# cshizhe/VLN-HAMT

Hardware: AMD Instinct MI355X
Metric: panorama-steps/sec, R2R proxy pretrain (36x768 views, 80-tok instr) (higher is better)
Workload: dtype bf16; 1 GPU; R2R 6-proxy-task pretrain step (fwd+bwd+clip+AdamW, dropout 0.1), fixed ViT features, R2R-canon model 174.8M params; per_gpu_batch=64, global_batch=64, txt_len=80, hist_len=5, views=36, task_mix=mlm:sap:sar:sprel:mrc:itm=5:1:1:1:2:2, parallelism=dp1, launch=hipGraph replay, dead_code_elimination=True

## Files before the change

include/hamt.h:

```cpp
#ifndef HAMT_H
#define HAMT_H

#include <stddef.h>
#include <stdint.h>

#ifdef __cplusplus
extern "C" {
#endif

#define HAMT_ABI_VERSION 2

typedef enum { HAMT_OK = 0, HAMT_ERR_ARG = -1, HAMT_ERR_UNSUPPORTED = -2, HAMT_ERR_LAUNCH = -3 } hamt_status;
typedef enum { HAMT_F32 = 0, HAMT_BF16 = 1,
               HAMT_U8G = 2,
               HAMT_F16 = 3 } hamt_dtype;
typedef enum { HAMT_PREC_BF16 = 0, HAMT_PREC_F32 = 1 } hamt_prec;

int hamt_version(void);
int hamt_last_error(char* buf, size_t n);
int hamt_last_kernel(char* buf, size_t n);
enum { HAMT_WS_GEMM_SPLITK = 0, HAMT_WS_COLSUM = 1, HAMT_WS_SUMSQ = 2, HAMT_WS_LN_BWD = 3, HAMT_WS_WGRAD_TABLE = 4, HAMT_WS_LNRED_TABLE = 5, HAMT_WS_VIS_EMBED_BWD = 6,
       HAMT_WS_EMBED_BWD = 7 ,
       HAMT_WS_OBJ_EMBED_BWD = 8, HAMT_WS_IMAGE_PREP = 9  };
size_t hamt_workspace_bytes(int op, const int* shape, int nshape);

enum {
  HAMT_EPI_BIAS = 1, HAMT_EPI_GELU = 2, HAMT_EPI_RELU = 4, HAMT_EPI_ACCUM = 8,
  HAMT_EPI_MUL_DGELU = 16, HAMT_EPI_MUL_DRELU = 32, HAMT_EPI_SAVE_PRE = 64,
  HAMT_EPI_GELU_GRAD = 128, HAMT_EPI_MUL_AUX = 256,
  HAMT_EPI_ADD_AUX = 512,
  HAMT_EPI_DROPOUT = 1024
};
typedef struct {
  int M, N, K;
  int lda, ldb, ldc, ldaux;
  int a_kmajor, b_kmajor;
  int dtype_a, dtype_b, dtype_c, dtype_aux;
  int prec;
  int epilogue;
  float alpha;
  int ka_rows, kb_rows;
  float p_drop;
  uint32_t call_id;
  const uint64_t* rng;
} hamt_gemm_desc;
int hamt_gemm(const hamt_gemm_desc* d, const void* A, const void* B, void* C, const float* bias,
              void* aux, void* stream);
int hamt_gemm_ksplit(const hamt_gemm_desc* d);
int hamt_gemm_ws(const hamt_gemm_desc* d, const void* A, const void* B, void* C, const float* bias,
                 void* aux, void* ws, size_t ws_bytes, void* stream);
int hamt_gemm_plan(const hamt_gemm_desc* d, size_t ws_bytes, char* name, size_t n);

int hamt_cast_pad_bf16(int R, int C, int Rpad, int Cpad, const float* x, int ldx, void* y, int ldy, void* stream);
int hamt_cast_transpose(int R, int C, const void* x, int ldx, int dtype_x, void* y, int ldy, int Rpad, void* stream);
int hamt_cast_pad_bf16_dropout(int R, int C, int Rpad, const float* x, int ldx, void* y, int ldy, float p, uint32_t call_id,
                               const uint64_t* rng, void* stream);

int hamt_smallk_wgrad(int M, int N, int K, const float* dy, int lddy, const float* x, int ldx, float* dW,
                      int accumulate, float* ws, void* stream);

typedef struct {
  const void* dy;
  const void* x;
  float* dw;
  float* db;
  int M, N, K, ldy, ldx, ldw;
  int accum_dw, accum_db;
  float* ss;
  int K_valid;
  float wire_scale;
  const void* dy2;
  const void* x2;
  int K2, ldy2, ldx2, K2_valid;
} hamt_wgrad_desc;
#define HAMT_WGRAD_TABLE_ENTRY 112
int hamt_wgrad_grouped(int n, const hamt_wgrad_desc* probs, void* table, size_t table_bytes, void* stream);
int hamt_wgrad_grouped_ex(int n, const hamt_wgrad_desc* probs, void* table, size_t table_bytes, int phase, void* stream);

int hamt_colsum(int M, int N, const void* x, int ldx, int dtype_x, float* out, int accumulate,
                float* ws, void* stream);

typedef struct {
  int B, heads, Sq, Sk, d_head;
  int ldq, ldk, ldv, ldo;
// ... 292 lines not shown
```

vln_hamt_amd/_lib.py:

```python
from __future__ import annotations

import ctypes as C
import os

_HERE = os.path.dirname(os.path.abspath(__file__))
LIB_PATH = os.path.join(_HERE, "libhamt_hip.so")

HAMT_F32, HAMT_BF16, HAMT_U8G, HAMT_F16 = 0, 1, 2, 3
PREC_BF16, PREC_F32 = 0, 1
EPI_BIAS, EPI_GELU, EPI_RELU, EPI_ACCUM, EPI_MUL_DGELU, EPI_MUL_DRELU, EPI_SAVE_PRE = 1, 2, 4, 8, 16, 32, 64
EPI_GELU_GRAD, EPI_MUL_AUX, EPI_ADD_AUX, EPI_DROPOUT = 128, 256, 512, 1024
SUMSQ_SPARSE = 2
OPT_ADAMW, OPT_ADAM, OPT_RMSPROP, OPT_SGD = 0, 1, 2, 3

vp, i32, u32, f32, sz = C.c_void_p, C.c_int, C.c_uint32, C.c_float, C.c_size_t


class GemmDesc(C.Structure):
    _fields_ = [("M", i32), ("N", i32), ("K", i32), ("lda", i32), ("ldb", i32), ("ldc", i32), ("ldaux", i32),
                ("a_kmajor", i32), ("b_kmajor", i32), ("dtype_a", i32), ("dtype_b", i32), ("dtype_c", i32),
                ("dtype_aux", i32), ("prec", i32), ("epilogue", i32), ("alpha", f32), ("ka_rows", i32), ("kb_rows", i32),
                ("p_drop", f32), ("call_id", u32), ("rng", C.c_void_p)]


# ... 47 lines not shown
    _fields_ = [("src", C.c_int32), ("left", C.c_int32), ("top", C.c_int32), ("width", C.c_int32), ("height", C.c_int32), ("flip", C.c_int32),
                ("zero", C.c_int32), ("order", C.c_int32), ("brightness", f32), ("contrast", f32), ("saturation", f32), ("reserved", C.c_int32)]


class ImagePrepDesc(C.Structure):
    _fields_ = [("n", i32), ("n_src", i32), ("H", i32), ("W", i32), ("layout", i32), ("ldy", i32), ("dtype_y", i32), ("Rpad", i32)]


RESAMPLE_BICUBIC, RESAMPLE_LANCZOS = 0, 1


class ImageResampleDesc(C.Structure):
    _fields_ = [(n, i32) for n in ("n", "H", "W", "OH", "OW", "x0", "y0", "w", "h", "filter", "kx", "ky")]


WGRAD_TABLE_ENTRY = 112


class WgradDesc(C.Structure):
    _fields_ = [("dy", vp), ("x", vp), ("dw", vp), ("db", vp), ("M", i32), ("N", i32), ("K", i32), ("ldy", i32),
                ("ldx", i32), ("ldw", i32), ("accum_dw", i32), ("accum_db", i32), ("ss", vp), ("K_valid", i32),
                ("wire_scale", f32), ("dy2", vp), ("x2", vp), ("K2", i32), ("ldy2", i32), ("ldx2", i32), ("K2_valid", i32)]


SIGNATURES = {
    "hamt_version": [],
    "hamt_last_error": [C.c_char_p, sz],
    "hamt_last_kernel": [C.c_char_p, sz],
    "hamt_workspace_bytes": [i32, C.POINTER(i32), i32],
    "hamt_gemm": [C.POINTER(GemmDesc), vp, vp, vp, vp, vp, vp],
    "hamt_gemm_ksplit": [C.POINTER(GemmDesc)],
    "hamt_gemm_ws": [C.POINTER(GemmDesc), vp, vp, vp, vp, vp, vp, sz, vp],
    "hamt_gemm_plan": [C.POINTER(GemmDesc), sz, C.c_char_p, sz],
    "hamt_cast_pad_bf16": [i32, i32, i32, i32, vp, i32, vp, i32, vp],
    "hamt_cast_pad_bf16_dropout": [i32, i32, i32, vp, i32, vp, i32, f32, u32, vp, vp],
    "hamt_cast_transpose": [i32, i32, vp, i32, i32, vp, i32, i32, vp],
    "hamt_wgrad_grouped": [i32, C.POINTER(WgradDesc), vp, sz, vp],
    "hamt_wgrad_grouped_ex": [i32, C.POINTER(WgradDesc), vp, sz, i32, vp],
    "hamt_smallk_wgrad": [i32, i32, i32, vp, i32, vp, i32, vp, i32, vp, vp],
    "hamt_colsum": [i32, i32, vp, i32, i32, vp, i32, vp, vp],
    "hamt_attn_small_fwd": [C.POINTER(AttnDesc), vp, vp, vp, vp, vp, vp, vp, vp],
    "hamt_attn_small_bwd": [C.POINTER(AttnDesc), vp, vp, vp, vp, vp, vp, vp, vp, vp, vp, vp, vp, vp],
    "hamt_attn_cls_fwd": [C.POINTER(AttnDesc), vp, vp, vp, vp, vp],
    "hamt_attn_varlen_fwd": [C.POINTER(AttnDesc), vp, vp, vp, vp, vp, vp, vp, vp],
    "hamt_attn_varlen_bwd": [C.POINTER(AttnDesc), vp, vp, vp, vp, vp, vp, vp, vp, vp, vp, vp, vp],
    "hamt_attn_varlen_cross_fwd": [C.POINTER(AttnDesc), vp, vp, vp, vp, vp, C.c_int, vp, vp, vp, vp, vp, vp],
    "hamt_attn_varlen_cross_bwd": [C.POINTER(AttnDesc), vp, vp, vp, vp, vp, C.c_int, vp, vp, vp, vp, vp, vp, vp, vp, vp, vp],
    "hamt_vis_embed_fwd": [C.POINTER(VisEmbedDesc)] + [vp] * 12,
    "hamt_vis_embed_bwd": [C.POINTER(VisEmbedDesc)] + [vp] * 18,
    "hamt_obj_embed_fwd": [C.POINTER(ObjEmbedDesc), C.POINTER(ObjEmbedParams)] + [vp] * 7,
    "hamt_obj_embed_bwd": [C.POINTER(ObjEmbedDesc), C.POINTER(ObjEmbedParams), C.POINTER(ObjEmbedGrads)] + [vp] * 10,
    "hamt_ln_fwd": [C.POINTER(LnDesc), vp, vp, vp, vp, vp, vp, vp, vp, vp, vp, vp],
    "hamt_ln_bwd": [C.POINTER(LnDesc), vp, vp, vp, vp, vp, vp, vp, vp, vp, vp, vp, vp, vp, vp],
    "hamt_ln_bwd_add": [C.POINTER(LnDesc), vp, vp, vp, vp, vp, vp, vp, vp, vp, vp, vp],
    "hamt_ln_bwd_reduce": [i32, i32, vp, vp, vp, vp, vp],
    "hamt_ln_bwd_reduce_grouped": [i32, vp, vp, sz, vp],
    "hamt_gather_rows": [i32, i32, vp, i32, vp, vp, i32, vp, i32, i32, vp],
    "hamt_scatter_add_rows": [i32, i32, vp, i32, i32, vp, vp, i32, vp],
    "hamt_scatter_add_rows_small": [i32, i32, vp, i32, i32, vp, i32, vp, vp, vp],
    "hamt_scatter_add_rows_ordered": [i32, i32, vp, i32, i32, vp, vp, i32, i32, vp, vp],
    "hamt_embed_sum_fwd": [i32, i32, i32, vp, vp, vp, vp, vp, vp],
    "hamt_embed_sum_bwd": [i32, i32, i32, i32, vp, vp, vp, vp, vp, vp, sz, vp],
    "hamt_mean_mid_fwd": [i32, i32, i32, vp, vp, vp],
    "hamt_mean_mid_bwd": [i32, i32, i32, vp, vp, vp],
    "hamt_mul_bcast_fwd": [i32, i32, i32, vp, vp, i32, vp, vp],
    "hamt_mul_bcast_bwd": [i32, i32, i32, vp, vp, i32, vp, vp, vp, vp],
# ... 67 lines not shown
        raise HamtError(f"{LIB_PATH} is missing: build it with `python vln_hamt_amd/csrc/build.py` "
                        "(there is no CPU/PyTorch fallback for the HAMT kernels)")
    import torch
    lib = C.CDLL(LIB_PATH)
    for name, args in SIGNATURES.items():
        fn = getattr(lib, name)
        fn.argtypes = args
        fn.restype = sz if name == "hamt_workspace_bytes" else i32
    if lib.hamt_version() != 2:
        raise HamtError("libhamt_hip.so ABI version mismatch")
    _lib = lib
    return lib


def last_error() -> str:
    buf = C.create_string_buffer(512)
    load().hamt_last_error(buf, 512)
    return buf.value.decode(errors="replace")


def last_kernel() -> str:
    buf = C.create_string_buffer(160)
    load().hamt_last_kernel(buf, 160)
    return buf.value.decode(errors="replace")


def gemm_plan(desc: GemmDesc, ws_bytes=None):
    buf = C.create_string_buffer(160)
    ks = load().hamt_gemm_plan(C.byref(desc), sz(-1).value if ws_bytes is None else ws_bytes, buf, 160)
    check(min(ks, 0), "hamt_gemm_plan")
    return ks, buf.value.decode(errors="replace")


def workspace_bytes(op: int, *shape) -> int:
    arr = (i32 * max(1, len(shape)))(*shape)
    return int(load().hamt_workspace_bytes(op, arr, len(shape)))


WS_GEMM_SPLITK, WS_COLSUM, WS_SUMSQ, WS_LN_BWD, WS_WGRAD_TABLE, WS_LNRED_TABLE, WS_VIS_EMBED_BWD, WS_EMBED_BWD, WS_OBJ_EMBED_BWD = range(9)
WS_IMAGE_PREP = 9


def check(rc: int, name: str):
    if rc != 0:
        raise HamtError(f"{name} failed (status {rc}): {last_error()}")
```

vln_hamt_amd/csrc/gemm.hip:

```cpp
#include "common.h"
#include "gemm_plan.h"

namespace {

struct GemmArgs {
  int M, N, K, lda, ldb;
  int ka_lim, kb_lim;
  int ldc, ldaux;
  int dtype_c, dtype_aux, epi;
  float alpha;
  const void* A;
  const void* B;
  void* C;
  const float* bias;
  void* aux;
};

__device__ __forceinline__ void epi_store(const GemmArgs& g, int row, int col, float acc) {
  if (row >= g.M || col >= g.N) return;
  float v = acc * g.alpha;
  if (g.epi & HAMT_EPI_BIAS) v += g.bias[col];
  size_t ia = (size_t)row * g.ldaux + col;
  if (g.epi & HAMT_EPI_SAVE_PRE) {
    if (g.dtype_aux == HAMT_BF16) ((bf16_t*)g.aux)[ia] = f2bf(v); else ((float*)g.aux)[ia] = v;
  }
  if (g.epi & HAMT_EPI_GELU) v = gelu_erf(v);
  if (g.epi & HAMT_EPI_GELU_GRAD) {
    float gg, dg;
    gelu_and_grad(v, gg, dg);
    v = gg;
    if (g.dtype_aux == HAMT_U8G) { const float d4[4] = {dg, 0.f, 0.f, 0.f}; ((uint8_t*)g.aux)[ia] = (uint8_t)(g8_pack4(d4) & 0xffu); }
    else if (g.dtype_aux == HAMT_BF16) ((bf16_t*)g.aux)[ia] = f2bf(dg); else ((float*)g.aux)[ia] = dg;
  }
  if (g.epi & HAMT_EPI_MUL_AUX)
    v *= g.dtype_aux == HAMT_U8G ? __builtin_fmaf((float)((const uint8_t*)g.aux)[ia], 0.005f, -0.13f)
                                 : ((g.dtype_aux == HAMT_BF16) ? bf2f(((const bf16_t*)g.aux)[ia]) : ((const float*)g.aux)[ia]);
  if (g.epi & HAMT_EPI_RELU) v = fmaxf(v, 0.0f);
  if (g.epi & (HAMT_EPI_MUL_DGELU | HAMT_EPI_MUL_DRELU)) {
    float h = (g.dtype_aux == HAMT_BF16) ? bf2f(((const bf16_t*)g.aux)[ia]) : ((const float*)g.aux)[ia];
    v *= (g.epi & HAMT_EPI_MUL_DGELU) ? dgelu_erf(h) : (h > 0.0f ? 1.0f : 0.0f);
  }
  if (g.epi & HAMT_EPI_ADD_AUX) v += (g.dtype_aux == HAMT_BF16) ? bf2f(((const bf16_t*)g.aux)[ia]) : ((const float*)g.aux)[ia];
  size_t ic = (size_t)row * g.ldc + col;
  if (g.dtype_c == HAMT_BF16) {
    bf16_t* c = (bf16_t*)g.C;
    if (g.epi & HAMT_EPI_ACCUM) v += bf2f(c[ic]);
    c[ic] = f2bf(v);
  } else if (g.dtype_c == HAMT_F16) {
    bf16_t* c = (bf16_t*)g.C;
    if (g.epi & HAMT_EPI_ACCUM) v += h2f(c[ic]);
    c[ic] = f2h(v);
  } else {
    float* c = (float*)g.C;
    if (g.epi & HAMT_EPI_ACCUM) v += c[ic];
    c[ic] = v;
  }
}

constexpr int F_BM = 64, F_BN = 64, F_BK = 32, F_LD = 64 + 16, F_NP = F_BK / 16;

template <bool KMAJOR>
__device__ __forceinline__ void f32_stage_load(const float* __restrict__ P, int ld, int r0, int rlim, int k0,
                                               int klim, int t, float (&v)[4]) {
  if (!KMAJOR) {
    int r = r0 + (t & 63), k = k0 + (t >> 6) * 4;
    if (r < rlim && k + 4 <= klim) {
      float4 x = *(const float4*)(P + (size_t)r * ld + k);
      v[0] = x.x; v[1] = x.y; v[2] = x.z; v[3] = x.w;
    } else {
#pragma unroll
      for (int j = 0; j < 4; ++j) v[j] = (r < rlim && k + j < klim) ? P[(size_t)r * ld + k + j] : 0.0f;
    }
  } else {
    int k = k0 + (t >> 4), r = r0 + (t & 15) * 4;
    if (k < klim && r + 4 <= rlim) {
      float4 x = *(const float4*)(P + (size_t)k * ld + r);
      v[0] = x.x; v[1] = x.y; v[2] = x.z; v[3] = x.w;
    } else {
#pragma unroll
      for (int j = 0; j < 4; ++j) v[j] = (k < klim && r + j < rlim) ? P[(size_t)k * ld + r + j] : 0.0f;
    }
  }
}
template <bool KMAJOR>
__device__ __forceinline__ void f32_stage_write(float* lds, int t, const float (&v)[4]) {
  if (!KMAJOR) {
    int r = t & 63, k = (t >> 6) * 4;
#pragma unroll
    for (int j = 0; j < 4; ++j) lds[(k + j) * F_LD + r] = v[j];
  } else {
    int k = t >> 4, r = (t & 15) * 4;
    *(float4*)(lds + k * F_LD + r) = make_float4(v[0], v[1], v[2], v[3]);
  }
}

template <bool A_KM, bool B_KM>
__global__ __launch_bounds__(256) void gemm_f32_kernel(GemmArgs g) {
  __shared__ __attribute__((aligned(16))) float lds[2][2][F_BK * F_LD];
  const int t = threadIdx.x, lane = t & 63, w = t >> 6, wm = w >> 1, wn = w & 1;
  const int tiles_n = (g.N + F_BN - 1) / F_BN;
  const int m0 = (blockIdx.x / tiles_n) * F_BM, n0 = (blockIdx.x % tiles_n) * F_BN;
  const float* A = (const float*)g.A;
  const float* B = (const float*)g.B;
  f32x4 acc[2][2];
#pragma unroll
  for (int i = 0; i < 2; ++i)
#pragma unroll
    for (int j = 0; j < 2; ++j) acc[i][j] = (f32x4){0.f, 0.f, 0.f, 0.f};

  float ra[F_NP][4], rb[F_NP][4];
  const int nk = (g.K + F_BK - 1) / F_BK;
#pragma unroll
  for (int h = 0; h < F_NP; ++h) {
    f32_stage_load<A_KM>(A, g.lda, m0, g.M, 16 * h, g.ka_lim, t, ra[h]);
    f32_stage_load<B_KM>(B, g.ldb, n0, g.N, 16 * h, g.kb_lim, t, rb[h]);
  }
#pragma unroll
  for (int h = 0; h < F_NP; ++h) {
    f32_stage_write<A_KM>(lds[0][0] + 16 * h * F_LD, t, ra[h]);
    f32_stage_write<B_KM>(lds[0][1] + 16 * h * F_LD, t, rb[h]);
  }
  __syncthreads();
  for (int kt = 0; kt < nk; ++kt) {
    const int cur = kt & 1;
    if (kt + 1 < nk) {
#pragma unroll
      for (int h = 0; h < F_NP; ++h) {
        f32_stage_load<A_KM>(A, g.lda, m0, g.M, (kt + 1) * F_BK + 16 * h, g.ka_lim, t, ra[h]);
        f32_stage_load<B_KM>(B, g.ldb, n0, g.N, (kt + 1) * F_BK + 16 * h, g.kb_lim, t, rb[h]);
      }
    }
    const float* As = lds[cur][0];
    const float* Bs = lds[cur][1];
#pragma unroll
    for (int s = 0; s < F_BK / 4; ++s) {
      const int kk = s * 4 + (lane >> 4);
      float a[2], b[2];
#pragma unroll
      for (int i = 0; i < 2; ++i) a[i] = As[kk * F_LD + wm * 32 + i * 16 + (lane & 15)];
#pragma unroll
      for (int j = 0; j < 2; ++j) b[j] = Bs[kk * F_LD + wn * 32 + j * 16 + (lane & 15)];
#pragma unroll
      for (int i = 0; i < 2; ++i)
#pragma unroll
        for (int j = 0; j < 2; ++j) acc[i][j] = __builtin_amdgcn_mfma_f32_16x16x4f32(a[i], b[j], acc[i][j], 0, 0, 0);
    }
    if (kt + 1 < nk) {
#pragma unroll
      for (int h = 0; h < F_NP; ++h) {
        f32_stage_write<A_KM>(lds[cur ^ 1][0] + 16 * h * F_LD, t, ra[h]);
        f32_stage_write<B_KM>(lds[cur ^ 1][1] + 16 * h * F_LD, t, rb[h]);
      }
    }
    __syncthreads();
  }
#pragma unroll
  for (int i = 0; i < 2; ++i)
#pragma unroll
    for (int j = 0; j < 2; ++j)
#pragma unroll
      for (int r = 0; r < 4; ++r)
        epi_store(g, m0 + wm * 32 + i * 16 + (lane >> 4) * 4 + r, n0 + wn * 32 + j * 16 + (lane & 15), acc[i][j][r]);
}

constexpr int H_BK = 32, H_PAD = 8;

template <typename T> struct Ld8;
template <> struct Ld8<float> {
  static __device__ __forceinline__ uint4 vec(const float* p) {
    float4 a = *(const float4*)p, b = *(const float4*)(p + 4);
    return make_uint4(pack_bf2(a.x, a.y), pack_bf2(a.z, a.w), pack_bf2(b.x, b.y), pack_bf2(b.z, b.w));
  }
  static __device__ __forceinline__ bf16_t one(const float* p) { return f2bf(*p); }
};
template <> struct Ld8<bf16_t> {
  static __device__ __forceinline__ uint4 vec(const bf16_t* p) { return *(const uint4*)p; }
  static __device__ __forceinline__ bf16_t one(const bf16_t* p) { return *p; }
};

template <typename T, bool KMAJOR, int R>
__device__ __forceinline__ uint4 h_stage_load(const T* __restrict__ P, int ld, int r0, int rlim, int k0, int klim, int c) {
  int r, k;
  const T* p;
  bool full;
  if (!KMAJOR) {
    r = r0 + (c >> 2); k = k0 + (c & 3) * 8;
    p = P + (size_t)r * ld + k;
    full = (r < rlim) && (k + 8 <= klim);
  } else {
    k = k0 + c / (R / 8); r = r0 + (c % (R / 8)) * 8;
    p = P + (size_t)k * ld + r;
    full = (k < klim) && (r + 8 <= rlim);
  }
  if (full) return Ld8<T>::vec(p);
  unsigned short e[8];
// ... 187 lines not shown
}

extern "C" int hamt_smallk_wgrad(int M, int N, int K, const float* dy, int lddy, const float* x, int ldx, float* dW, int accumulate,
                                 float* ws, void* stream) {
  HAMT_CHECK_ARG(dy && x && dW && ws && K >= 1 && K <= 8 && N >= 1 && M >= 0, "hamt_smallk_wgrad: bad argument (K <= 8)");
  hipStream_t s = as_stream(stream);
  int chunks = M >= 64 * 64 ? 64 : (M + 63) / 64;
  if (chunks < 1) chunks = 1;
  int rpc = (M + chunks - 1) / chunks;
  if (rpc < 1) rpc = 1;
  hipLaunchKernelGGL((smallk_wgrad_partial_kernel<8>), dim3((N + 63) / 64, chunks), dim3(256), 0, s, M, N, K, dy, lddy, x, ldx, ws, rpc);
  hamt_reduce_partials(chunks, N * K, ws, dW, accumulate, s);
  HAMT_CHECK_LAUNCH("hamt_smallk_wgrad");
  return HAMT_OK;
}

void hamt_gemm_fast_launch(const hamt_gemm_desc* d, const GemmPlan& p, const void* A, const void* B, void* C, const float* bias, void* aux,
                           float* ws, hipStream_t s);

void hamt_reduce_partials(int R, int N, const float* ws, float* out, int accumulate, hipStream_t s) {
  if (N % 4 == 0 && (((uintptr_t)ws | (uintptr_t)out) % 16) == 0) {
    const size_t n4 = (size_t)N / 4;
    const size_t b = (n4 + 255) / 256;
    hipLaunchKernelGGL(reduce_partials4_kernel, dim3((unsigned)(b > 4096 ? 4096 : b)), dim3(256), 0, s, R, n4, (size_t)N, ws, out, accumulate);
    return;
  }
  hipLaunchKernelGGL(reduce_partials_kernel, dim3((N + 63) / 64), dim3(256), 0, s, R, N, ws, out, accumulate);
}

static const GemmTuning& gemm_tuning() {
  static const GemmTuning t = [] {
    auto num = [](const char* name, int unset) { const char* v = getenv(name); return v ? atoi(v) : unset; };
    return GemmTuning{getenv("HAMT_NO_FAST") != nullptr, num("HAMT_FAST_BM", 0), num("HAMT_KS", 0), num("HAMT_KG", 0), num("HAMT_Q4", -1),
                      num("HAMT_P8", -1), num("HAMT_P8_BN", 0)};
  }();
  return t;
}

extern "C" int hamt_gemm_ksplit(const hamt_gemm_desc* d) { return d ? gemm_plan(*d, (size_t)-1, gemm_tuning()).ksplit : 1; }

extern "C" int hamt_gemm_plan(const hamt_gemm_desc* d, size_t ws_bytes, char* name, size_t n) {
  HAMT_CHECK_ARG(d && (name || n == 0), "hamt_gemm_plan: null pointer");
  const GemmPlan p = gemm_plan(*d, ws_bytes, gemm_tuning());
  if (n) gemm_plan_name(p, name, n);
  return p.ksplit;
}

extern "C" int hamt_gemm(const hamt_gemm_desc* d, const void* A, const void* B, void* C, const float* bias, void* aux,
                         void* stream) {
  return hamt_gemm_ws(d, A, B, C, bias, aux, nullptr, 0, stream);
}

extern "C" int hamt_gemm_ws(const hamt_gemm_desc* d, const void* A, const void* B, void* C, const float* bias, void* aux,
                            void* ws, size_t ws_bytes, void* stream) {
  HAMT_CHECK_ARG(d && A && B && C, "hamt_gemm: null pointer");
  HAMT_CHECK_ARG(d->M >= 0 && d->N >= 0 && d->K >= 0, "hamt_gemm: negative size");
  if (d->M == 0 || d->N == 0) return HAMT_OK;
  const int sa = d->dtype_a == HAMT_BF16 ? 2 : 4, sb = d->dtype_b == HAMT_BF16 ? 2 : 4;
  HAMT_CHECK_ARG((d->lda * sa) % 16 == 0 && (d->ldb * sb) % 16 == 0, "hamt_gemm: lda/ldb rows must be 16-byte aligned (lda=%d ldb=%d)", d->lda, d->ldb);
  HAMT_CHECK_ARG(((uintptr_t)A % 16) == 0 && ((uintptr_t)B % 16) == 0, "hamt_gemm: A/B must be 16-byte aligned");
  HAMT_CHECK_ARG(d->dtype_c == HAMT_F32 || d->dtype_c == HAMT_BF16 || d->dtype_c == HAMT_F16, "hamt_gemm: dtype_c = %d (C is fp32, bf16 or IEEE half)", d->dtype_c);
  HAMT_CHECK_ARG(d->dtype_c != HAMT_F16 || (d->epilogue & ~(HAMT_EPI_BIAS | HAMT_EPI_ACCUM)) == 0, "hamt_gemm: an IEEE-half C (HAMT_F16) takes the plain / bias / accumulate epilogues only");
  HAMT_CHECK_ARG((d->dtype_a == HAMT_F32 || d->dtype_a == HAMT_BF16) && (d->dtype_b == HAMT_F32 || d->dtype_b == HAMT_BF16), "hamt_gemm: operands are fp32 or bf16");
  HAMT_CHECK_ARG(!(d->epilogue & HAMT_EPI_BIAS) || bias, "hamt_gemm: EPI_BIAS without bias");
  HAMT_CHECK_ARG(!(d->epilogue & (HAMT_EPI_SAVE_PRE | HAMT_EPI_MUL_DGELU | HAMT_EPI_MUL_DRELU | HAMT_EPI_GELU_GRAD | HAMT_EPI_MUL_AUX | HAMT_EPI_ADD_AUX)) || aux, "hamt_gemm: epilogue needs aux");
  if (aux && d->dtype_aux == HAMT_U8G)
    HAMT_CHECK_ARG((d->epilogue & (HAMT_EPI_GELU_GRAD | HAMT_EPI_MUL_AUX)) && !(d->epilogue & (HAMT_EPI_SAVE_PRE | HAMT_EPI_MUL_DGELU | HAMT_EPI_MUL_DRELU | HAMT_EPI_ADD_AUX | HAMT_EPI_DROPOUT)),
                   "hamt_gemm: a HAMT_U8G aux is the gelu' image of HAMT_EPI_GELU_GRAD (without dropout) / HAMT_EPI_MUL_AUX only");
  const GemmPlan p = gemm_plan(*d, ws ? ws_bytes : 0, gemm_tuning());
  const bool fast = p.family != GEMM_F32 && p.family != GEMM_BF16;
  if (d->epilogue & HAMT_EPI_DROPOUT) {
    HAMT_CHECK_ARG(d->rng && d->p_drop >= 0.0f && d->p_drop < 1.0f, "hamt_gemm: EPI_DROPOUT needs rng and 0 <= p_drop < 1");
    HAMT_CHECK_ARG(fast, "hamt_gemm: EPI_DROPOUT is implemented by the bf16 MFMA path only (bf16 operands, K %% 64 == 0)");
  }
  const int ka = (d->ka_rows > 0 && d->ka_rows < d->K) ? d->ka_rows : d->K, kb = (d->kb_rows > 0 && d->kb_rows < d->K) ? d->kb_rows : d->K;
  GemmArgs g{d->M, d->N, d->K, d->lda, d->ldb, ka, kb, d->ldc, d->ldaux, d->dtype_c, d->dtype_aux, d->epilogue, d->alpha, A, B, C, bias, aux};
  hipStream_t s = as_stream(stream);
  char name[160];
  gemm_plan_name(p, name, sizeof(name));
  hamt_set_last_kernel("%s", name);
  if (fast) {
    hamt_gemm_fast_launch(d, p, A, B, C, bias, aux, (float*)ws, s);
    HAMT_CHECK_LAUNCH("hamt_gemm(fast)");
    return HAMT_OK;
  }
  if (d->prec == HAMT_PREC_F32) {
    HAMT_CHECK_ARG(d->dtype_a == HAMT_F32 && d->dtype_b == HAMT_F32, "hamt_gemm: PREC_F32 needs fp32 operands");
    int tiles = ((d->M + F_BM - 1) / F_BM) * ((d->N + F_BN - 1) / F_BN);
    if (!d->a_kmajor && !d->b_kmajor) hipLaunchKernelGGL((gemm_f32_kernel<false, false>), dim3(tiles), dim3(256), 0, s, g);
    else if (!d->a_kmajor && d->b_kmajor) hipLaunchKernelGGL((gemm_f32_kernel<false, true>), dim3(tiles), dim3(256), 0, s, g);
    else if (d->a_kmajor && !d->b_kmajor) hipLaunchKernelGGL((gemm_f32_kernel<true, false>), dim3(tiles), dim3(256), 0, s, g);
    else hipLaunchKernelGGL((gemm_f32_kernel<true, true>), dim3(tiles), dim3(256), 0, s, g);
  } else {
    static const bool use_tr = getenv("HAMT_NO_TR") == nullptr;
    static const int force_tile = getenv("HAMT_GEMM_TILE") ? atoi(getenv("HAMT_GEMM_TILE")) : 0;
    if (!d->a_kmajor && !d->b_kmajor) pick_types_bf16<false, false>(g, d->dtype_a, d->dtype_b, use_tr, force_tile, s);
    else if (!d->a_kmajor && d->b_kmajor) pick_types_bf16<false, true>(g, d->dtype_a, d->dtype_b, use_tr, force_tile, s);
    else if (d->a_kmajor && d->b_kmajor) pick_types_bf16<true, true>(g, d->dtype_a, d->dtype_b, use_tr, force_tile, s);
    else { hamt_set_error("hamt_gemm: a_kmajor=1,b_kmajor=0 is not used by the path"); return HAMT_ERR_UNSUPPORTED; }
  }
  HAMT_CHECK_LAUNCH("hamt_gemm");
  return HAMT_OK;
}

extern "C" int hamt_colsum(int M, int N, const void* x, int ldx, int dtype_x, float* out, int accumulate, float* ws,
                           void* stream) {
  HAMT_CHECK_ARG(x && out && ws && M >= 0 && N > 0, "hamt_colsum: bad argument");
  hipStream_t s = as_stream(stream);
  int chunks = M >= 64 * 64 ? 64 : (M + 63) / 64;
  if (chunks < 1) chunks = 1;
  int rpc = (M + chunks - 1) / chunks;
  if (rpc < 1) rpc = 1;
  dim3 grid((N + 63) / 64, chunks);
  if (dtype_x == HAMT_BF16) hipLaunchKernelGGL((colsum_partial_kernel<bf16_t>), grid, dim3(256), 0, s, M, N, (const bf16_t*)x, ldx, ws, rpc);
  else hipLaunchKernelGGL((colsum_partial_kernel<float>), grid, dim3(256), 0, s, M, N, (const float*)x, ldx, ws, rpc);
  hamt_reduce_partials(chunks, N, ws, out, accumulate, s);
  HAMT_CHECK_LAUNCH("hamt_colsum");
  return HAMT_OK;
}
```

vln_hamt_amd/csrc/gemm_plan.h:

```cpp
#pragma once
#include "../../include/hamt.h"
#include <stddef.h>
#include <stdio.h>

constexpr int PLAN_BN = 128, PLAN_BK = 64;

#define HAMT_EPIS_NARROW(X) X(0) X(HAMT_EPI_BIAS) X(HAMT_EPI_ACCUM)
#define HAMT_EPIS_P8(X) HAMT_EPIS_NARROW(X) X(HAMT_EPI_BIAS | HAMT_EPI_GELU_GRAD) X(HAMT_EPI_MUL_AUX)
#define HAMT_EPIS_P8_FWD(X)  \
  X(HAMT_EPI_BIAS | HAMT_EPI_ADD_AUX) X(HAMT_EPI_BIAS | HAMT_EPI_ADD_AUX | HAMT_EPI_DROPOUT) X(HAMT_EPI_BIAS | HAMT_EPI_GELU_GRAD | HAMT_EPI_DROPOUT) \
  X(HAMT_EPI_BIAS | HAMT_EPI_GELU) X(HAMT_EPI_BIAS | HAMT_EPI_GELU | HAMT_EPI_DROPOUT)
#define HAMT_EPIS_256(X) HAMT_EPIS_P8(X)  \
  X(HAMT_EPI_BIAS | HAMT_EPI_ADD_AUX) X(HAMT_EPI_BIAS | HAMT_EPI_ADD_AUX | HAMT_EPI_DROPOUT) X(HAMT_EPI_BIAS | HAMT_EPI_GELU_GRAD | HAMT_EPI_DROPOUT)
#define HAMT_EPIS_FAST(X) HAMT_EPIS_P8(X) HAMT_EPIS_P8_FWD(X)  \
  X(HAMT_EPI_BIAS | HAMT_EPI_GELU | HAMT_EPI_SAVE_PRE) X(HAMT_EPI_BIAS | HAMT_EPI_RELU) X(HAMT_EPI_MUL_DGELU)
#define HAMT_KG_VARIANTS(X) X(32, 2, 3) X(32, 3, 2) X(32, 2, 4) X(64, 2, 3) X(64, 3, 2) X(128, 2, 2)

#define HAMT_EPI_IS(E) if (e == (E)) return true;
static inline bool gemm_epi_narrow(int e) { HAMT_EPIS_NARROW(HAMT_EPI_IS) return false; }
static inline bool gemm_epi_256(int e) { HAMT_EPIS_256(HAMT_EPI_IS) return false; }
static inline bool gemm_epi_fast(int e) { HAMT_EPIS_FAST(HAMT_EPI_IS) return false; }
static inline bool gemm_epi_p8(int e, bool b_kmajor, int nb) {
  HAMT_EPIS_P8(HAMT_EPI_IS)
  if (!b_kmajor && nb == 4) { HAMT_EPIS_P8_FWD(HAMT_EPI_IS) }
  return false;
}
#undef HAMT_EPI_IS

struct GemmTuning {
  bool no_fast;
  int fast_bm;
  int ks;
  int kg;
  int q4, p8;
  int p8_bn;
};

enum GemmFamily { GEMM_F32, GEMM_BF16 , GEMM_FAST, GEMM_FAST256, GEMM_P8, GEMM_KG, GEMM_Q4 };

struct GemmPlan {
  GemmFamily family;
  int tile_rows;
  int p8_nb;
  int kg_groups, kg_depth;
  int epi;
  bool a_kmajor, b_kmajor;
  int ksplit;
};

static inline int gemm_plan_name(const GemmPlan& p, char* buf, size_t n) {
  const char *a = p.a_kmajor ? "true" : "false", *b = p.b_kmajor ? "true" : "false";
  switch (p.family) {
    case GEMM_F32: return snprintf(buf, n, "gemm_f32_kernel<%s, %s>", a, b);
    case GEMM_BF16: return snprintf(buf, n, "gemm_bf16_kernel<%s, %s, ...>", a, b);
    case GEMM_FAST: return snprintf(buf, n, "gemm_fast_kernel<%d, %d, %s, %s>", p.tile_rows, p.epi, a, b);
    case GEMM_FAST256: return snprintf(buf, n, "gemm_fast256_kernel<%d, %s, %s>", p.epi, a, b);
    case GEMM_P8: return snprintf(buf, n, "gemm_p8_kernel<%d, %s, %s, %d>", p.epi, a, b, p.p8_nb);
    case GEMM_KG: return snprintf(buf, n, "gemm_kg_kernel<%d, %d, %d, %s>", p.tile_rows, p.kg_groups, p.kg_depth, b);
    case GEMM_Q4: return snprintf(buf, n, "gemm_q4_kernel<%d, %s>", p.epi, b);
  }
  return -1;
}

static inline bool gemm_fast_eligible(const hamt_gemm_desc& d) {
  if (d.prec != HAMT_PREC_BF16 || d.dtype_a != HAMT_BF16 || d.dtype_b != HAMT_BF16) return false;
  if (d.a_kmajor && !d.b_kmajor) return false;
  if (d.K < 64 || d.M < 1 || d.N < 1) return false;
  if (d.K % 64 != 0) return false;
// ... 16 lines not shown
    if (bm == 32) return G == 2 && D == 3 ? GemmKg{32, 2, 3} : G == 3 ? GemmKg{32, 3, 2} : GemmKg{32, 2, 4};
    if (bm == 128) return {128, 2, 2};
    return G == 2 ? GemmKg{64, 2, 3} : GemmKg{64, 3, 2};
  }
  const int nk = d.K / PLAN_BK;
  if (nk < 12 || d.N > 1024) return {0, 0, 0};
  const long tn = (d.N + 127) / 128, t32 = (long)((d.M + 31) / 32) * tn, t64 = (long)((d.M + 63) / 64) * tn;
  if (nk >= 192 && t64 <= 128 && !(d.epilogue & ~HAMT_EPI_ACCUM) && d.dtype_c == HAMT_F32 && d.ldc == d.N) return {0, 0, 0};
  if (t32 <= 256) return {32, 2, 4};
  if (t64 <= 256 && nk >= 24) return {64, 3, 2};
  const long t128 = (long)((d.M + 127) / 128) * tn;
  if (t128 <= 256 && nk >= 36) return {128, 2, 2};
  return {0, 0, 0};
}

static inline int gemm_ksplit(const hamt_gemm_desc& d, size_t ws_bytes, const GemmTuning& t) {
  if (d.epilogue & ~HAMT_EPI_ACCUM) return 1;
  if (d.dtype_c != HAMT_F32 || d.ldc != d.N) return 1;
  if (!t.fast_bm && !t.ks && gemm_kg_variant(d, t).rows) return 1;
  const long tiles = (long)((d.M + 127) / 128) * ((d.N + 127) / 128);
  const int nk = d.K / PLAN_BK;
  int s;
  if (t.ks) s = t.ks > nk ? nk : t.ks;
  else {
    if (tiles >= 192 || nk < 16) return 1;
    s = (int)(384 / tiles);
    if (s > nk / 8) s = nk / 8;
    if (s > 16) s = 16;
  }
  while (s > 1 && (size_t)s * d.M * d.N * 4 > ws_bytes) --s;
  return s < 2 ? 1 : s;
}

static inline GemmPlan gemm_plan(const hamt_gemm_desc& d, size_t ws_bytes, const GemmTuning& t) {
  GemmPlan p{GEMM_BF16, 0, 0, 0, 0, -1, d.a_kmajor != 0, d.b_kmajor != 0, 1};
  if (t.no_fast || !gemm_fast_eligible(d)) {
    if (d.prec == HAMT_PREC_F32) p.family = GEMM_F32;
    return p;
  }
  const int e = d.epilogue, nk = d.K / PLAN_BK;
  const int ks = p.ksplit = gemm_ksplit(d, ws_bytes, t);
  const long t128 = (long)((d.M + 127) / 128) * ((d.N + 127) / 128), t64 = (long)((d.M + 63) / 64) * ((d.N + 127) / 128);
  const bool one_tile = ks == 1 && !t.fast_bm;
  if (one_tile && t.q4 != 0 && !d.a_kmajor && nk >= 3 && gemm_epi_narrow(e)) {
    if (t.q4 == 1 || (d.N <= 1024 && d.K >= 192 && t128 >= 120 && t128 <= 256)) { p.family = GEMM_Q4; p.epi = e; return p; }
  }
  if (one_tile && t.p8 != 0 && d.K >= 128 && !d.a_kmajor && (!d.b_kmajor || d.ldb >= 256)) {
    const long t256 = (long)((d.M + 255) / 256) * ((d.N + 255) / 256), t192 = (long)((d.M + 255) / 256) * ((d.N + 191) / 192);
    const double t_p8 = (double)((t256 + 255) / 256) * (6.0 + 1.55 * nk);
    const double t_p8n = (double)((t192 + 255) / 256) * (6.0 + 1.44 * nk);
    const bool n192 = t.p8_bn ? t.p8_bn == 192 : (t_p8n < 0.97 * t_p8 && !((e & HAMT_EPI_GELU_GRAD) && t192 > 512));
    const double t_small = 2.0 * d.M * d.N * d.K / 620e6;
    if (t.p8 == 1 || (n192 ? t_p8n : t_p8) < 0.95 * t_small) {
      const int nb = n192 && gemm_epi_p8(e, p.b_kmajor, 3) ? 3 : 4;
      if (gemm_epi_p8(e, p.b_kmajor, nb)) { p.family = GEMM_P8; p.p8_nb = nb; p.epi = e; return p; }
    }
  }
  if (one_tile) {
    const GemmKg kg = gemm_kg_variant(d, t);
    if (kg.rows) { p.family = GEMM_KG; p.tile_rows = kg.rows; p.kg_groups = kg.groups; p.kg_depth = kg.depth; return p; }
  }
  if (ks == 1 && !d.a_kmajor && !(d.b_kmajor && d.ldb < 256) && gemm_epi_256(e)) {
    const long t256 = (long)((d.M + 255) / 256) * ((d.N + 255) / 256);
    if (t.fast_bm ? t.fast_bm == 256 : (d.K >= 2048 && ((t256 >= 208 && t256 <= 256) || t256 >= 768))) { p.family = GEMM_FAST256; p.epi = e; return p; }
  }
  const long r128 = (t128 * ks + 511) / 512, r64 = (t64 * ks + 767) / 768;
// ... 8 lines not shown
```

Baseline: 6299 panorama-steps/s.

## Add 32x32 register-ring fp32 GEMM kernel for small-tile-count fp32 GEMMs

Adds a new fp32 MFMA GEMM kernel with 32x32 tiles and a two-deep register/LDS ring that prefetches two K-steps ahead, selected when the 64x64 tile count is low or K is tiny. This targets poor occupancy and exposed load latency on small fp32 GEMMs. It also relaxes the alignment requirement for fp32 operands by adding a non-vectorised load path, and exposes the tile choice through a new API and env knob. The extra kernel variants raise code size, and the smaller tiles reuse less data per load.

```diff
diff --git a/include/hamt.h b/include/hamt.h
--- a/include/hamt.h
+++ b/include/hamt.h
@@ -50,6 +50,7 @@
 int hamt_gemm_ws(const hamt_gemm_desc* d, const void* A, const void* B, void* C, const float* bias,
                  void* aux, void* ws, size_t ws_bytes, void* stream);
 int hamt_gemm_plan(const hamt_gemm_desc* d, size_t ws_bytes, char* name, size_t n);
+int hamt_gemm_f32_tile(const hamt_gemm_desc* d, int aligned, int* bm, int* bn, int* bk);
 
 int hamt_cast_pad_bf16(int R, int C, int Rpad, int Cpad, const float* x, int ldx, void* y, int ldy, void* stream);
 int hamt_cast_transpose(int R, int C, const void* x, int ldx, int dtype_x, void* y, int ldy, int Rpad, void* stream);
diff --git a/vln_hamt_amd/_lib.py b/vln_hamt_amd/_lib.py
--- a/vln_hamt_amd/_lib.py
+++ b/vln_hamt_amd/_lib.py
@@ -103,6 +103,7 @@
     "hamt_gemm_ksplit": [C.POINTER(GemmDesc)],
     "hamt_gemm_ws": [C.POINTER(GemmDesc), vp, vp, vp, vp, vp, vp, sz, vp],
     "hamt_gemm_plan": [C.POINTER(GemmDesc), sz, C.c_char_p, sz],
+    "hamt_gemm_f32_tile": [C.POINTER(GemmDesc), i32, C.POINTER(i32), C.POINTER(i32), C.POINTER(i32)],
     "hamt_cast_pad_bf16": [i32, i32, i32, i32, vp, i32, vp, i32, vp],
     "hamt_cast_pad_bf16_dropout": [i32, i32, i32, vp, i32, vp, i32, f32, u32, vp, vp],
     "hamt_cast_transpose": [i32, i32, vp, i32, i32, vp, i32, i32, vp],
@@ -236,6 +237,12 @@
     return ks, buf.value.decode(errors="replace")
 
 
+def gemm_f32_tile(desc: GemmDesc, aligned=True):
+    bm, bn, bk = i32(), i32(), i32()
+    check(load().hamt_gemm_f32_tile(C.byref(desc), int(aligned), C.byref(bm), C.byref(bn), C.byref(bk)), "hamt_gemm_f32_tile")
+    return bm.value, bn.value, bk.value
+
+
 def workspace_bytes(op: int, *shape) -> int:
     arr = (i32 * max(1, len(shape)))(*shape)
     return int(load().hamt_workspace_bytes(op, arr, len(shape)))
diff --git a/vln_hamt_amd/csrc/gemm.hip b/vln_hamt_amd/csrc/gemm.hip
--- a/vln_hamt_amd/csrc/gemm.hip
+++ b/vln_hamt_amd/csrc/gemm.hip
@@ -14,6 +14,7 @@
   void* C;
   const float* bias;
   void* aux;
+  int vec;
 };
 
 __device__ __forceinline__ void epi_store(const GemmArgs& g, int row, int col, float acc) {
@@ -60,11 +61,9 @@
 constexpr int F_BM = 64, F_BN = 64, F_BK = 32, F_LD = 64 + 16, F_NP = F_BK / 16;
 
 template <bool KMAJOR>
-__device__ __forceinline__ void f32_stage_load(const float* __restrict__ P, int ld, int r0, int rlim, int k0,
-                                               int klim, int t, float (&v)[4]) {
+__device__ __forceinline__ void f32_chunk_load(const float* __restrict__ P, int ld, int r, int rlim, int k, int klim, bool vec, float (&v)[4]) {
   if (!KMAJOR) {
-    int r = r0 + (t & 63), k = k0 + (t >> 6) * 4;
-    if (r < rlim && k + 4 <= klim) {
+    if (vec && r < rlim && k + 4 <= klim) {
       float4 x = *(const float4*)(P + (size_t)r * ld + k);
       v[0] = x.x; v[1] = x.y; v[2] = x.z; v[3] = x.w;
     } else {
@@ -72,8 +71,7 @@
       for (int j = 0; j < 4; ++j) v[j] = (r < rlim && k + j < klim) ? P[(size_t)r * ld + k + j] : 0.0f;
     }
   } else {
-    int k = k0 + (t >> 4), r = r0 + (t & 15) * 4;
-    if (k < klim && r + 4 <= rlim) {
+    if (vec && k < klim && r + 4 <= rlim) {
       float4 x = *(const float4*)(P + (size_t)k * ld + r);
       v[0] = x.x; v[1] = x.y; v[2] = x.z; v[3] = x.w;
     } else {
@@ -81,6 +79,12 @@
       for (int j = 0; j < 4; ++j) v[j] = (k < klim && r + j < rlim) ? P[(size_t)k * ld + r + j] : 0.0f;
     }
   }
+}
+template <bool KMAJOR>
+__device__ __forceinline__ void f32_stage_load(const float* __restrict__ P, int ld, int r0, int rlim, int k0,
+                                               int klim, int t, bool vec, float (&v)[4]) {
+  if (!KMAJOR) f32_chunk_load<false>(P, ld, r0 + (t & 63), rlim, k0 + (t >> 6) * 4, klim, vec, v);
+  else f32_chunk_load<true>(P, ld, r0 + (t & 15) * 4, rlim, k0 + (t >> 4), klim, vec, v);
 }
 template <bool KMAJOR>
 __device__ __forceinline__ void f32_stage_write(float* lds, int t, const float (&v)[4]) {
@@ -102,6 +106,7 @@
   const int m0 = (blockIdx.x / tiles_n) * F_BM, n0 = (blockIdx.x % tiles_n) * F_BN;
   const float* A = (const float*)g.A;
   const float* B = (const float*)g.B;
+  const bool vec = g.vec != 0;
   f32x4 acc[2][2];
 #pragma unroll
   for (int i = 0; i < 2; ++i)
@@ -112,8 +117,8 @@
   const int nk = (g.K + F_BK - 1) / F_BK;
 #pragma unroll
   for (int h = 0; h < F_NP; ++h) {
-    f32_stage_load<A_KM>(A, g.lda, m0, g.M, 16 * h, g.ka_lim, t, ra[h]);
-    f32_stage_load<B_KM>(B, g.ldb, n0, g.N, 16 * h, g.kb_lim, t, rb[h]);
+    f32_stage_load<A_KM>(A, g.lda, m0, g.M, 16 * h, g.ka_lim, t, vec, ra[h]);
+    f32_stage_load<B_KM>(B, g.ldb, n0, g.N, 16 * h, g.kb_lim, t, vec, rb[h]);
   }
 #pragma unroll
   for (int h = 0; h < F_NP; ++h) {
@@ -126,8 +131,8 @@
     if (kt + 1 < nk) {
 #pragma unroll
       for (int h = 0; h < F_NP; ++h) {
-        f32_stage_load<A_KM>(A, g.lda, m0, g.M, (kt + 1) * F_BK + 16 * h, g.ka_lim, t, ra[h]);
-        f32_stage_load<B_KM>(B, g.ldb, n0, g.N, (kt + 1) * F_BK + 16 * h, g.kb_lim, t, rb[h]);
+        f32_stage_load<A_KM>(A, g.lda, m0, g.M, (kt + 1) * F_BK + 16 * h, g.ka_lim, t, vec, ra[h]);
+        f32_stage_load<B_KM>(B, g.ldb, n0, g.N, (kt + 1) * F_BK + 16 * h, g.kb_lim, t, vec, rb[h]);
       }
     }
     const float* As = lds[cur][0];
@@ -161,6 +166,158 @@
 #pragma unroll
       for (int r = 0; r < 4; ++r)
         epi_store(g, m0 + wm * 32 + i * 16 + (lane >> 4) * 4 + r, n0 + wn * 32 + j * 16 + (lane & 15), acc[i][j][r]);
+}
+
+template <bool KMAJOR, bool WHOLE>
+__device__ __forceinline__ void f32_chunk_load_nb(const float* __restrict__ P, int ld, int r, int rlim, int k, int klim, float (&v)[4]) {
+  const size_t idx = KMAJOR ? (size_t)k * ld + r : (size_t)r * ld + k;
+  if (WHOLE) {
+    const bool ok = r < rlim && k < klim;
+    const float4 x = *(const float4*)(P + (ok ? idx : (size_t)0));
+    v[0] = x.x; v[1] = x.y; v[2] = x.z; v[3] = x.w;
+  } else {
+#pragma unroll
+    for (int j = 0; j < 4; ++j) {
+      const bool ok = KMAJOR ? (k < klim && r + j < rlim) : (r < rlim && k + j < klim);
+      v[j] = P[ok ? idx + j : (size_t)0];
+    }
+  }
+}
+template <bool KMAJOR, bool WHOLE>
+__device__ __forceinline__ void f32_chunk_mask(int r, int rlim, int k, int klim, float (&v)[4]) {
+#pragma unroll
+  for (int j = 0; j < 4; ++j) {
+    const bool ok = WHOLE ? (r < rlim && k < klim) : KMAJOR ? (k < klim && r + j < rlim) : (r < rlim && k + j < klim);
+    v[j] = ok ? v[j] : 0.0f;
+  }
+}
+__device__ __forceinline__ bool f32_ring_whole(bool kmajor, int r0, int R, int rlim, int klim) {
+  return kmajor ? (rlim % 4 == 0 || r0 + R <= rlim) : klim % 4 == 0;
+}
+
+template <bool KMAJOR, int R>
+struct F32Ring {
+  static constexpr int LD = R + 16, CH = R * F_BK / 4 / 256;
+  static_assert(R == 32 || R == 64, "tile");
+  template <bool WHOLE>
+  static __device__ __forceinline__ void load(const float* __restrict__ P, int ld, int r0, int rlim, int k0, int klim, int t, float (&v)[CH][4]) {
+#pragma unroll
+    for (int q = 0; q < CH; ++q) {
+      const int c = t + q * 256;
+      if (!KMAJOR) f32_chunk_load_nb<false, WHOLE>(P, ld, r0 + c % R, rlim, k0 + (c / R) * 4, klim, v[q]);
+      else f32_chunk_load_nb<true, WHOLE>(P, ld, r0 + (c % (R / 4)) * 4, rlim, k0 + c / (R / 4), klim, v[q]);
+    }
+  }
+  template <bool WHOLE>
+  static __device__ __forceinline__ void write(float* lds, int r0, int rlim, int k0, int klim, int t, float (&v)[CH][4]) {
+#pragma unroll
+    for (int q = 0; q < CH; ++q) {
+      const int c = t + q * 256;
+      if (!KMAJOR) {
+        f32_chunk_mask<false, WHOLE>(r0 + c % R, rlim, k0 + (c / R) * 4, klim, v[q]);
+#pragma unroll
+        for (int j = 0; j < 4; ++j) lds[((c / R) * 4 + j) * LD + c % R] = v[q][j];
+      } else {
+        f32_chunk_mask<true, WHOLE>(r0 + (c % (R / 4)) * 4, rlim, k0 + c / (R / 4), klim, v[q]);
+        *(float4*)(lds + (c / (R / 4)) * LD + (c % (R / 4)) * 4) = make_float4(v[q][0], v[q][1], v[q][2], v[q][3]);
+      }
+    }
+  }
+};
+
+template <int FR, int LD>
+__device__ __forceinline__ void f32_ring_mfma(const float* As, const float* Bs, int lane, f32x4 (&acc)[FR][FR]) {
+#pragma unroll
+  for (int s = 0; s < F_BK / 4; ++s) {
+    const int kk = s * 4 + (lane >> 4);
+    float a[FR], b[FR];
+#pragma unroll
+    for (int i = 0; i < FR; ++i) a[i] = As[kk * LD + i * 16 + (lane & 15)];
+#pragma unroll
+    for (int j = 0; j < FR; ++j) b[j] = Bs[kk * LD + j * 16 + (lane & 15)];
+#pragma unroll
+    for (int i = 0; i < FR; ++i)
+#pragma unroll
+      for (int j = 0; j < FR; ++j) acc[i][j] = __builtin_amdgcn_mfma_f32_16x16x4f32(a[i], b[j], acc[i][j], 0, 0, 0);
+  }
+}
+
+template <int FR, bool A_KM, bool B_KM, bool WHOLE>
+__device__ __forceinline__ void f32_ring_walk(const GemmArgs& g, float* lds, int m0, int n0, f32x4 (&acc)[FR][FR]) {
+  constexpr int BT = 32 * FR, BK = F_BK;
+  using SA = F32Ring<A_KM, BT>;
+  using SB = F32Ring<B_KM, BT>;
+  constexpr int LD = BT + 16, SZ = BK * LD;
+  const int t = threadIdx.x, lane = t & 63, w = t >> 6, wm = w >> 1, wn = w & 1;
+  const float* A = (const float*)g.A;
+  const float* B = (const float*)g.B;
+  const int nk = (g.K + BK - 1) / BK;
+  float* const L0 = lds;
+  float* const L1 = lds + 2 * SZ;
+  const float* const Af0 = L0 + wm * (16 * FR), * const Bf0 = L0 + SZ + wn * (16 * FR);
+  const float* const Af1 = L1 + wm * (16 * FR), * const Bf1 = L1 + SZ + wn * (16 * FR);
+  float ra0[SA::CH][4], rb0[SB::CH][4], ra1[SA::CH][4], rb1[SB::CH][4];
+  SA::template load<WHOLE>(A, g.lda, m0, g.M, 0, g.ka_lim, t, ra0);
+  SB::template load<WHOLE>(B, g.ldb, n0, g.N, 0, g.kb_lim, t, rb0);
+  SA::template load<WHOLE>(A, g.lda, m0, g.M, BK, g.ka_lim, t, ra1);
+  SB::template load<WHOLE>(B, g.ldb, n0, g.N, BK, g.kb_lim, t, rb1);
+  SA::template write<WHOLE>(L0, m0, g.M, 0, g.ka_lim, t, ra0);
+  SB::template write<WHOLE>(L0 + SZ, n0, g.N, 0, g.kb_lim, t, rb0);
+  __syncthreads();
+  for (int kt = 0; kt < nk; kt += 2) {
+    SA::template load<WHOLE>(A, g.lda, m0, g.M, (kt + 2) * BK, g.ka_lim, t, ra0);
+    SB::template load<WHOLE>(B, g.ldb, n0, g.N, (kt + 2) * BK, g.kb_lim, t, rb0);
+    __builtin_amdgcn_sched_barrier(0);
+    f32_ring_mfma<FR, LD>(Af0, Bf0, lane, acc);
+    __builtin_amdgcn_sched_barrier(0);
+    SA::template write<WHOLE>(L1, m0, g.M, (kt + 1) * BK, g.ka_lim, t, ra1);
+    SB::template write<WHOLE>(L1 + SZ, n0, g.N, (kt + 1) * BK, g.kb_lim, t, rb1);
+    __syncthreads();
+    if (kt + 1 >= nk) break;
+    SA::template load<WHOLE>(A, g.lda, m0, g.M, (kt + 3) * BK, g.ka_lim, t, ra1);
+    SB::template load<WHOLE>(B, g.ldb, n0, g.N, (kt + 3) * BK, g.kb_lim, t, rb1);
+    __builtin_amdgcn_sched_barrier(0);
+    f32_ring_mfma<FR, LD>(Af1, Bf1, lane, acc);
+    __builtin_amdgcn_sched_barrier(0);
+    SA::template write<WHOLE>(L0, m0, g.M, (kt + 2) * BK, g.ka_lim, t, ra0);
+    SB::template write<WHOLE>(L0 + SZ, n0, g.N, (kt + 2) * BK, g.kb_lim, t, rb0);
+    __syncthreads();
+  }
+}
+
+template <int FR, bool A_KM, bool B_KM>
+__global__ __launch_bounds__(256) void gemm_f32_ring_kernel(GemmArgs g) {
+  constexpr int BT = 32 * FR;
+  __shared__ __attribute__((aligned(16))) float lds[2 * 2 * F_BK * (BT + 16)];
+  const int lane = threadIdx.x & 63, w = threadIdx.x >> 6, wm = w >> 1, wn = w & 1;
+  const int tiles_n = (g.N + BT - 1) / BT;
+  const int m0 = (blockIdx.x / tiles_n) * BT, n0 = (blockIdx.x % tiles_n) * BT;
+  f32x4 acc[FR][FR];
+#pragma unroll
+  for (int i = 0; i < FR; ++i)
+#pragma unroll
+    for (int j = 0; j < FR; ++j) acc[i][j] = (f32x4){0.f, 0.f, 0.f, 0.f};
+  if (f32_ring_whole(A_KM, m0, BT, g.M, g.ka_lim) && f32_ring_whole(B_KM, n0, BT, g.N, g.kb_lim))
+    f32_ring_walk<FR, A_KM, B_KM, true>(g, lds, m0, n0, acc);
+  else
+    f32_ring_walk<FR, A_KM, B_KM, false>(g, lds, m0, n0, acc);
+#pragma unroll
+  for (int i = 0; i < FR; ++i)
+#pragma unroll
+    for (int j = 0; j < FR; ++j)
+#pragma unroll
+      for (int r = 0; r < 4; ++r)
+        epi_store(g, m0 + (wm * FR + i) * 16 + (lane >> 4) * 4 + r, n0 + (wn * FR + j) * 16 + (lane & 15), acc[i][j][r]);
+}
+
+template <int FR>
+void launch_f32_ring(const GemmArgs& g, bool a_km, bool b_km, hipStream_t s) {
+  const int tiles = ((g.M + 32 * FR - 1) / (32 * FR)) * ((g.N + 32 * FR - 1) / (32 * FR));
+  const dim3 grid(tiles), block(256);
+  if (!a_km && !b_km) hipLaunchKernelGGL((gemm_f32_ring_kernel<FR, false, false>), grid, block, 0, s, g);
+  else if (!a_km && b_km) hipLaunchKernelGGL((gemm_f32_ring_kernel<FR, false, true>), grid, block, 0, s, g);
+  else if (a_km && !b_km) hipLaunchKernelGGL((gemm_f32_ring_kernel<FR, true, false>), grid, block, 0, s, g);
+  else hipLaunchKernelGGL((gemm_f32_ring_kernel<FR, true, true>), grid, block, 0, s, g);
 }
 
 constexpr int H_BK = 32, H_PAD = 8;
@@ -414,7 +571,7 @@
   static const GemmTuning t = [] {
     auto num = [](const char* name, int unset) { const char* v = getenv(name); return v ? atoi(v) : unset; };
     return GemmTuning{getenv("HAMT_NO_FAST") != nullptr, num("HAMT_FAST_BM", 0), num("HAMT_KS", 0), num("HAMT_KG", 0), num("HAMT_Q4", -1),
-                      num("HAMT_P8", -1), num("HAMT_P8_BN", 0)};
+                      num("HAMT_P8", -1), num("HAMT_P8_BN", 0), num("HAMT_F32_TILE", 0)};
   }();
   return t;
 }
@@ -426,6 +583,17 @@
   const GemmPlan p = gemm_plan(*d, ws_bytes, gemm_tuning());
   if (n) gemm_plan_name(p, name, n);
   return p.ksplit;
+}
+
+static bool f32_operands_aligned(const hamt_gemm_desc* d, const void* A, const void* B) {
+  return d->lda % 4 == 0 && d->ldb % 4 == 0 && (((uintptr_t)A | (uintptr_t)B) % 16) == 0;
+}
+
+extern "C" int hamt_gemm_f32_tile(const hamt_gemm_desc* d, int aligned, int* bm, int* bn, int* bk) {
+  HAMT_CHECK_ARG(d && bm && bn && bk, "hamt_gemm_f32_tile: null pointer");
+  const GemmF32Tile t = gemm_f32_tile(*d, aligned != 0, gemm_tuning());
+  *bm = t.bm; *bn = t.bn; *bk = t.bk;
+  return HAMT_OK;
 }
 
 extern "C" int hamt_gemm(const hamt_gemm_desc* d, const void* A, const void* B, void* C, const float* bias, void* aux,
@@ -439,8 +607,9 @@
   HAMT_CHECK_ARG(d->M >= 0 && d->N >= 0 && d->K >= 0, "hamt_gemm: negative size");
   if (d->M == 0 || d->N == 0) return HAMT_OK;
   const int sa = d->dtype_a == HAMT_BF16 ? 2 : 4, sb = d->dtype_b == HAMT_BF16 ? 2 : 4;
-  HAMT_CHECK_ARG((d->lda * sa) % 16 == 0 && (d->ldb * sb) % 16 == 0, "hamt_gemm: lda/ldb rows must be 16-byte aligned (lda=%d ldb=%d)", d->lda, d->ldb);
-  HAMT_CHECK_ARG(((uintptr_t)A % 16) == 0 && ((uintptr_t)B % 16) == 0, "hamt_gemm: A/B must be 16-byte aligned");
+  const bool any_align = d->prec == HAMT_PREC_F32 && d->dtype_a == HAMT_F32 && d->dtype_b == HAMT_F32;
+  HAMT_CHECK_ARG(any_align || ((d->lda * sa) % 16 == 0 && (d->ldb * sb) % 16 == 0), "hamt_gemm: lda/ldb rows must be 16-byte aligned (lda=%d ldb=%d)", d->lda, d->ldb);
+  HAMT_CHECK_ARG(any_align || (((uintptr_t)A % 16) == 0 && ((uintptr_t)B % 16) == 0), "hamt_gemm: A/B must be 16-byte aligned");
   HAMT_CHECK_ARG(d->dtype_c == HAMT_F32 || d->dtype_c == HAMT_BF16 || d->dtype_c == HAMT_F16, "hamt_gemm: dtype_c = %d (C is fp32, bf16 or IEEE half)", d->dtype_c);
   HAMT_CHECK_ARG(d->dtype_c != HAMT_F16 || (d->epilogue & ~(HAMT_EPI_BIAS | HAMT_EPI_ACCUM)) == 0, "hamt_gemm: an IEEE-half C (HAMT_F16) takes the plain / bias / accumulate epilogues only");
   HAMT_CHECK_ARG((d->dtype_a == HAMT_F32 || d->dtype_a == HAMT_BF16) && (d->dtype_b == HAMT_F32 || d->dtype_b == HAMT_BF16), "hamt_gemm: operands are fp32 or bf16");
@@ -468,8 +637,11 @@
   }
   if (d->prec == HAMT_PREC_F32) {
     HAMT_CHECK_ARG(d->dtype_a == HAMT_F32 && d->dtype_b == HAMT_F32, "hamt_gemm: PREC_F32 needs fp32 operands");
+    g.vec = f32_operands_aligned(d, A, B);
+    const GemmF32Tile ft = gemm_f32_tile(*d, g.vec != 0, gemm_tuning());
     int tiles = ((d->M + F_BM - 1) / F_BM) * ((d->N + F_BN - 1) / F_BN);
-    if (!d->a_kmajor && !d->b_kmajor) hipLaunchKernelGGL((gemm_f32_kernel<false, false>), dim3(tiles), dim3(256), 0, s, g);
+    if (ft.bm == 32) launch_f32_ring<1>(g, d->a_kmajor != 0, d->b_kmajor != 0, s);
+    else if (!d->a_kmajor && !d->b_kmajor) hipLaunchKernelGGL((gemm_f32_kernel<false, false>), dim3(tiles), dim3(256), 0, s, g);
     else if (!d->a_kmajor && d->b_kmajor) hipLaunchKernelGGL((gemm_f32_kernel<false, true>), dim3(tiles), dim3(256), 0, s, g);
     else if (d->a_kmajor && !d->b_kmajor) hipLaunchKernelGGL((gemm_f32_kernel<true, false>), dim3(tiles), dim3(256), 0, s, g);
     else hipLaunchKernelGGL((gemm_f32_kernel<true, true>), dim3(tiles), dim3(256), 0, s, g);
diff --git a/vln_hamt_amd/csrc/gemm_plan.h b/vln_hamt_amd/csrc/gemm_plan.h
--- a/vln_hamt_amd/csrc/gemm_plan.h
+++ b/vln_hamt_amd/csrc/gemm_plan.h
@@ -34,6 +34,7 @@
   int kg;
   int q4, p8;
   int p8_bn;
+  int f32_tile;
 };
 
 enum GemmFamily { GEMM_F32, GEMM_BF16 , GEMM_FAST, GEMM_FAST256, GEMM_P8, GEMM_KG, GEMM_Q4 };
@@ -116,6 +117,14 @@
   return s < 2 ? 1 : s;
 }
 
+struct GemmF32Tile { int bm, bn, bk; };
+static inline GemmF32Tile gemm_f32_tile(const hamt_gemm_desc& d, bool aligned, const GemmTuning& t) {
+  if (!aligned || t.no_fast || d.K < 1) return {0, 0, 0};
+  const long t64 = (long)((d.M + 63) / 64) * ((d.N + 63) / 64);
+  const bool ring = t.f32_tile ? t.f32_tile == 32 : (t64 < 384 || d.K <= 32);
+  return ring ? GemmF32Tile{32, 32, 32} : GemmF32Tile{0, 0, 0};
+}
+
 static inline GemmPlan gemm_plan(const hamt_gemm_desc& d, size_t ws_bytes, const GemmTuning& t) {
   GemmPlan p{GEMM_BF16, 0, 0, 0, 0, -1, d.a_kmajor != 0, d.b_kmajor != 0, 1};
   if (t.no_fast || !gemm_fast_eligible(d)) {
```

Measured after the change: 6344 panorama-steps/s, median of 6. No clear change (+0.7%).
